# dangvansam/viet-asr

Hardware: AMD Instinct MI355X
Metric: real_time_factor (higher is better)
Workload: dtype f32 via 2xf16 split operands (22-bit significands, 3 f16 MFMA products per multiply, fp32 accumulate)

## Files before the change

viet-asr_amd/csrc/encoder_dw_mfma.hip:

```cpp
#include <cstdlib>

#include "vasr_internal.h"
#include "vasr_device.h"
#include <type_traits>

namespace vasr {

namespace {

using f32x4 = __attribute__((ext_vector_type(4))) float;
using v4f = __attribute__((ext_vector_type(4))) float;
using v2f = __attribute__((ext_vector_type(2))) float;
using f16x8 = __attribute__((ext_vector_type(8))) _Float16;
using f16x2 = __attribute__((ext_vector_type(2))) _Float16;
using u32x4 = __attribute__((vector_size(16))) unsigned int;

constexpr int kTile = 512;
constexpr int kGroup = 256;
constexpr int kUttPerWave = 8;
constexpr int kRowStages = 1;

template <int K, int DIL>
struct TzGeom {
  static constexpr int PAD = DIL > 1 ? (DIL * K) / 2 - 1 : K / 2;
  static constexpr int PADL = (PAD + 3) & ~3;
  static constexpr int OFF = PADL - PAD;
  static constexpr int SPAN = 15 + DIL * (K - 1) + OFF + 1;
  static constexpr int NS = (SPAN + 31) / 32;
  static constexpr int STAGES = kRowStages;
  static constexpr int TSZ = 32 * NS + 16;
  static constexpr int ROWS = kTile - 16 + 32 * NS;
  static constexpr int NLD = (ROWS / 4 + 63) / 64;
  static constexpr int PLANE = 2 * 256 * NLD;
  static constexpr int LDS_DATA = 2 * PLANE;
  static constexpr int LDS_TAB = 4 * TSZ;
  static constexpr int LDS_WAVE = LDS_DATA + LDS_TAB;
  static_assert(ROWS % 4 == 0 && LDS_WAVE % 16 == 0, "staging granularity");
};

__device__ __forceinline__ void wave_sync() {
  __builtin_amdgcn_fence(__ATOMIC_RELEASE, "wavefront");
  __builtin_amdgcn_wave_barrier();
  __builtin_amdgcn_fence(__ATOMIC_ACQUIRE, "wavefront");
}
__device__ __forceinline__ f32x4 mma(uint4 a, uint4 b, f32x4 c) {
  return __builtin_amdgcn_mfma_f32_16x16x32_f16(__builtin_bit_cast(f16x8, a), __builtin_bit_cast(f16x8, b), c, 0, 0, 0);
}
__device__ __forceinline__ float lane_pull(int src4, float v) {
  return __int_as_float(__builtin_amdgcn_ds_bpermute(src4, __float_as_int(v)));
}

template <int K, int DIL>
__global__ __launch_bounds__(256) void dw_toeplitz_kernel(const float* __restrict__ x, int64_t ldx,
                                                          const unsigned* __restrict__ taps,
                                                          const float* __restrict__ tap_inv,
                                                          const int32_t* __restrict__ lens_in,
                                                          const int32_t* __restrict__ lens_out,
                                                          const unsigned* __restrict__ amax_x, int amax_x_stride,
                                                          int amax_x_n, int channels, int batch,
                                                          float* __restrict__ y, int64_t ldy,
                                                          unsigned* __restrict__ amax_y, int amax_y_stride, int upw_nt,
                                                          int tiles, int n_rest) {
  using G = TzGeom<K, DIL>;
  const int bid = (int)blockIdx.x;
  const int rest = ((bid >> 3) / tiles) * 8 + (bid & 7);
  if (rest >= n_rest) return;
  const int ncg = channels >> 2;
  const int bx = rest % ncg, by = rest / ncg, bz = (bid >> 3) % tiles;
  const int upw = upw_nt;
  constexpr int NS = G::NS, NLD = G::NLD, kStages = G::STAGES;
  extern __shared__ __attribute__((aligned(16))) unsigned char lds_raw[];
  const int lane = threadIdx.x & 63;
  const int wave = __builtin_amdgcn_readfirstlane(threadIdx.x >> 6);
  unsigned char* base = lds_raw + wave * G::LDS_WAVE;
  unsigned char* dat = base;
  unsigned* tab = reinterpret_cast<unsigned*>(base + G::LDS_DATA);
  const int c = bx * 4 + wave;
  const int t_tile = bz * kTile;
  const int n16 = lane & 15, kg = lane >> 4;
  const int b_lo = by * upw;
  const int b_hi = min(b_lo + upw, batch);
  if (b_lo >= b_hi) return;
  const bool two = t_tile + kGroup < ldy;

  uint4 ah[NS], al[NS];
  const float w_inv = tap_inv[c];

  struct Stage { v4f r[NLD]; };
  const int n_ld = min(NLD, (min((int)ldy - t_tile, kTile) - 16 + 32 * NS + 255) / 256);
  int voff[NLD];
#pragma unroll
  for (int j = 0; j < NLD; ++j) {
    const int tau = 4 * (lane + 64 * j);
    voff[j] = tau < G::ROWS && j < n_ld ? 4 * (t_tile - G::PADL + tau) : (int)0x80000000u;
    if (j >= n_ld) {
      *reinterpret_cast<uint2*>(dat + 8 * lane + 512 * j) = make_uint2(0u, 0u);
      *reinterpret_cast<uint2*>(dat + G::PLANE + 8 * lane + 512 * j) = make_uint2(0u, 0u);
    }
  }
  const int n_utt = b_hi - b_lo;
  const int64_t row_stride = (int64_t)channels * ldx;
  const float* xrow0 = x + ((int64_t)b_lo * channels + c) * ldx;
  const int64_t yrow_stride = (int64_t)channels * ldy;
  float* yrow0 = y + ((int64_t)b_lo * channels + c) * ldy;
  int rng[kUttPerWave], lout[kUttPerWave];
#pragma unroll
  for (int u = 0; u < kUttPerWave; ++u) {
    const int b = min(b_lo + u, batch - 1);
    rng[u] = u < n_utt ? 4 * min(lens_in[b], (int)ldx) : 0;
    lout[u] = lens_out[b];
  }
  auto gload = [&](int u, Stage& sg) {
    const auto d = __builtin_amdgcn_make_buffer_rsrc(const_cast<float*>(xrow0 + u * row_stride), 0, rng[u], 0x00020000);
#pragma unroll
    for (int j = 0; j < NLD; ++j) {
      sg.r[j] = __builtin_bit_cast(v4f, __builtin_amdgcn_raw_buffer_load_b128(d, voff[j], 0, 0));
    }
  };
  auto sstore = [&](const Stage& sg, float sx) {
    unsigned char* ph = dat + 8 * lane;
#pragma unroll
    for (int j = 0; j < NLD; ++j) {
      if (j >= n_ld) continue;
      const v4f v = sg.r[j];
      const v2f a = {v.x * sx, v.y * sx}, b = {v.z * sx, v.w * sx};
      const f16x2 ha = __builtin_convertvector(a, f16x2), hb = __builtin_convertvector(b, f16x2);
      const f16x2 la = __builtin_convertvector(a - __builtin_convertvector(ha, v2f), f16x2);
      const f16x2 lb = __builtin_convertvector(b - __builtin_convertvector(hb, v2f), f16x2);
      *reinterpret_cast<uint2*>(ph + 512 * j) = make_uint2(__builtin_bit_cast(unsigned, ha), __builtin_bit_cast(unsigned, hb));
      *reinterpret_cast<uint2*>(ph + G::PLANE + 512 * j) = make_uint2(__builtin_bit_cast(unsigned, la), __builtin_bit_cast(unsigned, lb));
    }
  };

  const unsigned char* bb = dat + 32 * n16 + 16 * kg;
  const int pull = 4 * ((lane >> 2) + 16 * (lane & 3));
  const int slot = c * tiles + bz;

  float sxu[kUttPerWave], ixu[kUttPerWave];
  unsigned mxu[kUttPerWave];
#pragma unroll
  for (int u = 0; u < kUttPerWave; ++u) mxu[u] = 0u;
  auto publish = [&]() {
    if (!amax_y) return;
#define VASR_DPP(xx, ctrl) ((unsigned)__builtin_amdgcn_update_dpp(0, (int)(xx), (ctrl), 0xF, 0xF, false))
    const bool b0 = lane & 1, b1 = lane & 2, b2 = lane & 4;
    unsigned r[4], q[2];
#pragma unroll
    for (int k = 0; k < 4; ++k)
      r[k] = max(b0 ? mxu[2 * k + 1] : mxu[2 * k], VASR_DPP(b0 ? mxu[2 * k] : mxu[2 * k + 1], 0xB1));
#pragma unroll
    for (int k = 0; k < 2; ++k)
      q[k] = max(b1 ? r[2 * k + 1] : r[2 * k], VASR_DPP(b1 ? r[2 * k] : r[2 * k + 1], 0x4E));
    const unsigned send = b2 ? q[0] : q[1];
    unsigned m = max(b2 ? q[1] : q[0], max(VASR_DPP(send, 0x104), VASR_DPP(send, 0x114)));
    m = max(m, VASR_DPP(m, 0x128));
#undef VASR_DPP
    {
      const auto sw = __builtin_amdgcn_permlane16_swap(m, m, false, false);
      m = max((unsigned)sw[0], (unsigned)sw[1]);
    }
    {
      const auto sw = __builtin_amdgcn_permlane32_swap(m, m, false, false);
      m = max((unsigned)sw[0], (unsigned)sw[1]);
    }
    const auto da = __builtin_amdgcn_make_buffer_rsrc(amax_y + (int64_t)b_lo * amax_y_stride, 0, 4 * n_utt * amax_y_stride, 0x00020000);
    const int off = lane < kUttPerWave ? 4 * (lane * amax_y_stride + slot) : (int)0x80000000u;
    __builtin_amdgcn_raw_buffer_store_b32(m, da, off, 0, 0);
  };
  auto do_task = [&](auto u_tag, Stage& sg) {
    constexpr int u = decltype(u_tag)::value;
    sstore(sg, sxu[u]);
    if constexpr (u + kStages < kUttPerWave) gload(u + kStages, sg);
    wave_sync();

    f32x4 acc0 = {0.f, 0.f, 0.f, 0.f}, acc1 = {0.f, 0.f, 0.f, 0.f};
    constexpr bool kAllB = NS <= 3;
    auto load_b = [&](int q, uint4 (&bh)[NS], uint4 (&bl)[NS]) {
#pragma unroll
      for (int s = 0; s < NS; ++s) {
        bh[s] = *reinterpret_cast<const uint4*>(bb + 2 * kGroup * q + 64 * s);
        bl[s] = *reinterpret_cast<const uint4*>(bb + G::PLANE + 2 * kGroup * q + 64 * s);
      }
    };
    auto step = [&](f32x4 acc, int s, const uint4 (&bh)[NS], const uint4 (&bl)[NS]) {
      acc = mma(al[s], bh[s], acc);
      acc = mma(ah[s], bl[s], acc);
      acc = mma(ah[s], bh[s], acc);
      return acc;
    };
    {
      uint4 b0h[NS], b0l[NS], b1h[NS], b1l[NS];
      load_b(0, b0h, b0l);
      if (kAllB && two) {
        load_b(1, b1h, b1l);
#pragma unroll
        for (int s = 0; s < NS; ++s) {
          acc0 = step(acc0, s, b0h, b0l);
          acc1 = step(acc1, s, b1h, b1l);
        }
      } else {
#pragma unroll
        for (int s = 0; s < NS; ++s) acc0 = step(acc0, s, b0h, b0l);
        if (two) {
          load_b(1, b1h, b1l);
#pragma unroll
          for (int s = 0; s < NS; ++s) acc1 = step(acc1, s, b1h, b1l);
        }
      }
    }

    const float os = w_inv * ixu[u];
    const int lo = lout[u];
    float* yr = yrow0 + u * yrow_stride;
    const auto dy = __builtin_amdgcn_make_buffer_rsrc(yr, 0, 4 * (int)ldy, 0x00020000);
    v4f o0 = {acc0[0] * os, acc0[1] * os, acc0[2] * os, acc0[3] * os};
    v4f o1 = {acc1[0] * os, acc1[1] * os, acc1[2] * os, acc1[3] * os};
    o0.x = lane_pull(pull, o0.x); o0.y = lane_pull(pull, o0.y); o0.z = lane_pull(pull, o0.z); o0.w = lane_pull(pull, o0.w);
    o1.x = lane_pull(pull, o1.x); o1.y = lane_pull(pull, o1.y); o1.z = lane_pull(pull, o1.z); o1.w = lane_pull(pull, o1.w);
    float mx = 0.f;
    auto finish = [&](v4f o, int q) {
      const int tq = t_tile + kGroup * q;
      if (lo < tq + kGroup) {
        const int nv = lo - tq - 4 * lane;
        o.x = nv > 0 ? o.x : 0.f;
        o.y = nv > 1 ? o.y : 0.f;
        o.z = nv > 2 ? o.z : 0.f;
        o.w = nv > 3 ? o.w : 0.f;
      }
      mx = fmaxf(mx, fmaxf(fmaxf(fabsf(o.x), fabsf(o.y)), fmaxf(fabsf(o.z), fabsf(o.w))));
      __builtin_amdgcn_raw_buffer_store_b128(__builtin_bit_cast(u32x4, o), dy, 4 * (tq + 4 * lane), 0, 0);
    };
    finish(o0, 0);
    finish(o1, 1);
    mxu[u] = __float_as_uint(mx);
    wave_sync();
  };

  Stage stg[kStages];
#pragma unroll
  for (int i = 0; i < kStages; ++i) gload(i, stg[i]);

  constexpr int NTL = (G::TSZ + 63) / 64;
  unsigned tapv[NTL];
#pragma unroll
  for (int j = 0; j < NTL; ++j) tapv[j] = lane + 64 * j < G::TSZ ? taps[(int64_t)c * G::TSZ + lane + 64 * j] : 0u;

  {
    unsigned m[kUttPerWave];
    const unsigned* ap[kUttPerWave];
#pragma unroll
    for (int u = 0; u < kUttPerWave; ++u) {
      m[u] = 0u;
      ap[u] = amax_x + (int64_t)min(b_lo + u, b_hi - 1) * amax_x_stride;
    }
    for (int i0 = 0; i0 < amax_x_n; i0 += 64) {
      const int i = min(i0 + lane, amax_x_n - 1);
#pragma unroll
      for (int u = 0; u < kUttPerWave; ++u) m[u] = max(m[u], ap[u][i]);
    }
#pragma unroll
    for (int u = 0; u < kUttPerWave; ++u) f16_scale(wave_max_u32(m[u]), &sxu[u], &ixu[u]);
  }

#pragma unroll
  for (int j = 0; j < NTL; ++j)
    if (lane + 64 * j < G::TSZ) tab[lane + 64 * j] = tapv[j];
  wave_sync();
  {
    const unsigned* tp = tab + 15 - n16 + 8 * kg;
#pragma unroll
    for (int s = 0; s < NS; ++s) {
      unsigned v[8];
#pragma unroll
      for (int e = 0; e < 8; ++e) v[e] = tp[32 * s + e];
      ah[s] = make_uint4(__builtin_amdgcn_perm(v[1], v[0], 0x05040100u), __builtin_amdgcn_perm(v[3], v[2], 0x05040100u),
                         __builtin_amdgcn_perm(v[5], v[4], 0x05040100u), __builtin_amdgcn_perm(v[7], v[6], 0x05040100u));
      al[s] = make_uint4(__builtin_amdgcn_perm(v[1], v[0], 0x07060302u), __builtin_amdgcn_perm(v[3], v[2], 0x07060302u),
                         __builtin_amdgcn_perm(v[5], v[4], 0x07060302u), __builtin_amdgcn_perm(v[7], v[6], 0x07060302u));
    }
  }

  auto run = [&](auto u_tag, auto& self) -> void {
    constexpr int u = decltype(u_tag)::value;
    if constexpr (u < kUttPerWave) {
      if (u >= n_utt) return publish();
      do_task(u_tag, stg[u % kStages]);
      self(std::integral_constant<int, u + 1>{}, self);
    } else {
      publish();
    }
  };
  run(std::integral_constant<int, 0>{}, run);
}

template <int K, int DIL>
int launch_tz(const float* x, int64_t ldx, const unsigned* taps, const float* tap_inv, const int32_t* li, const int32_t* lo,
              AmaxTab amax_x, int batch, int channels, float* y, int64_t ldy, AmaxTab* amax_y, hipStream_t st) {
  using G = TzGeom<K, DIL>;
  auto kern = dw_toeplitz_kernel<K, DIL>;
  constexpr int lds = 4 * G::LDS_WAVE;
  const unsigned tiles = (unsigned)((ldy + kTile - 1) / kTile);
  const int upw_env = dev_switches().dw_upw;
  int upw = kUttPerWave;
  if (upw_env >= 1 && upw_env <= kUttPerWave) upw = upw_env;
  else
    while (upw > 2 && (int64_t)channels * ((batch + upw - 1) / upw) * tiles < 4096) upw /= 2;
  const int n_rest = (channels / 4) * ((batch + upw - 1) / upw);
  dim3 grid((unsigned)(((n_rest + 7) / 8) * 8) * tiles);
  if (amax_y) {
    amax_y->n = channels * (int)tiles;
    if (amax_y->n > amax_y->stride) return -1;
  }
  VASR_LAUNCH(kern, grid, dim3(256), lds, st, x, ldx, taps, tap_inv, li, lo, amax_x.p, amax_x.stride, amax_x.n, channels, batch,
              y, ldy, amax_y ? amax_y->p : nullptr, amax_y ? amax_y->stride : 0,
              upw, (int)tiles, n_rest);
  return 0;
}

template <int K, int DIL>
int table_size() { return TzGeom<K, DIL>::TSZ; }

}

int depthwise_mfma_table_size(int kernel, int dilation) {
  if (dilation == 2 && kernel == 87) return table_size<87, 2>();
  if (dilation != 1) return 0;
  switch (kernel) {
    case 33: return table_size<33, 1>();
    case 39: return table_size<39, 1>();
    case 51: return table_size<51, 1>();
    case 63: return table_size<63, 1>();
    case 75: return table_size<75, 1>();
    default: return 0;
  }
}

float pack_depthwise_taps_f16x2(const float* w, int kernel, int dilation, int tsz, unsigned* table) {
  const int pad = dilation > 1 ? (dilation * kernel) / 2 - 1 : kernel / 2;
  const int off = ((pad + 3) & ~3) - pad;
  float mx = 0.f;
  for (int k = 0; k < kernel; ++k) mx = fabsf(w[k]) > mx ? fabsf(w[k]) : mx;
  int e = (int)(__builtin_bit_cast(unsigned, mx) >> 23);
  e = e < 16 ? 16 : (e > 254 ? 254 : e);
  const float s = __builtin_bit_cast(float, (unsigned)(268 - e) << 23), inv = __builtin_bit_cast(float, (unsigned)(e - 14) << 23);
  for (int i = 0; i < tsz; ++i) {
    const int d = i - (15 + off);
    float v = 0.f;
    if (d >= 0 && d % dilation == 0 && d / dilation < kernel) v = w[d / dilation] * s;
    const _Float16 h = (_Float16)v;
    const _Float16 l = (_Float16)(v - (float)h);
    table[i] = (unsigned)__builtin_bit_cast(unsigned short, h) | ((unsigned)__builtin_bit_cast(unsigned short, l) << 16);
  }
  return inv;
}

int launch_depthwise_mfma(const float* x, int64_t ldx, const unsigned* taps, const float* tap_inv, const int32_t* lens_in,
                          const int32_t* lens_out, AmaxTab amax_x, int batch, int channels, int kernel, int dilation,
                          float* y, int64_t ldy, AmaxTab* amax_y, hipStream_t st) {
  const bool aligned = channels % 4 == 0 && ldx % 4 == 0 && ldy % 4 == 0 && ldx >= 4 &&
                       (reinterpret_cast<uintptr_t>(x) & 15) == 0 && (reinterpret_cast<uintptr_t>(y) & 15) == 0;
  if (!aligned || !taps || !amax_x.p || amax_x.n <= 0) return -1;
#define TZ(KK, DD) return launch_tz<KK, DD>(x, ldx, taps, tap_inv, lens_in, lens_out, amax_x, batch, channels, y, ldy, amax_y, st)
  if (dilation == 2 && kernel == 87) TZ(87, 2);
  if (dilation == 1) {
    switch (kernel) {
      case 33: TZ(33, 1);
      case 39: TZ(39, 1);
      case 51: TZ(51, 1);
      case 63: TZ(63, 1);
      case 75: TZ(75, 1);
      default: break;
    }
  }
#undef TZ
  return -1;
}

}
```

viet-asr_amd/csrc/vasr_api.cpp:

```cpp
#include <hip/hip_runtime.h>

#include <cmath>
#include <cstdarg>
#include <cstdio>
#include <cstdlib>
#include <cstring>
#include <map>
#include <string>
#include <algorithm>
#include <vector>

#include "vasr.h"
#include "vasr_devtools.h"
#include "vasr_internal.h"

using namespace vasr;

namespace vasr { thread_local LaunchProbe g_probe; }

namespace {

thread_local std::string g_err;

int fail(int code, const char* fmt, ...) {
  char buf[512];
  va_list ap;
  va_start(ap, fmt);
  vsnprintf(buf, sizeof buf, fmt, ap);
  va_end(ap);
  g_err = buf;
  return code;
}

#define HIP_TRY(expr)                                                                          \
  do {                                                                                         \
    hipError_t e_ = (expr);                                                                    \
    if (e_ != hipSuccess) return fail(VASR_ERR_HIP, "%s: %s", #expr, hipGetErrorString(e_)); \
  } while (0)

struct HostTensor {
  std::vector<float> data;
  std::vector<int64_t> shape;
};

struct ConvLayer {
  int cin = 0, cout = 0, kernel = 1, stride = 1, dilation = 1, pad = 0;
  int m_pad = 0;
  float* d_w = nullptr;
  unsigned short* d_w3 = nullptr;
  unsigned short* d_w16 = nullptr;
  float w16_inv = 1.f;
  unsigned int* d_taps = nullptr;
  float* d_tap_inv = nullptr;
  int tap_tsz = 0;
  float* d_ftaps = nullptr;
  float f_l1 = 0.f;
  float* d_scale = nullptr;
  float* d_shift = nullptr;
  int step = -1;
  int conv_cin = 0;
  int groups = 1;
};

struct SeLayer {
  float* d_w1 = nullptr;
  float* d_w2 = nullptr;
  int c = 0, hidden = 0;
};

struct NormLayer {
  float* d_gamma = nullptr;
  float* d_beta = nullptr;
  int32_t* d_group_of = nullptr;
  int32_t* d_members = nullptr;
  int c = 0, groups = 0;
};

struct SubBlock {
  bool separable = true;
  ConvLayer dw, pw;
  ConvLayer pw_bd;
  SeLayer se;
  NormLayer norm;
};

struct Block {
  vasr_block_desc d;
  std::vector<SubBlock> subs;
  bool has_res = false;
  ConvLayer res;
  bool fused_res = false;
  ConvLayer fused;
  int fused_k1 = 0;
  int first_step = 0;
  int pane = -1, pane_off = 0, pane_c = 0, dense_panes = 0;
  bool keep_input = false;
  bool res_pane0 = false;
  int se_r = 0;
  int groups = 1, heads = 0;
  int norm_g = 0;
  std::vector<NormLayer> res_norm;
  std::vector<SeLayer> res_se;
  std::vector<ConvLayer> res_panes;
  std::vector<int> res_pane_off;
};

size_t align_up(size_t v, size_t a) { return (v + a - 1) / a * a; }
constexpr int kDefaultGemmMode = 3;
int parse_gemm_mode(const char* s) {
  if (!s) return kDefaultGemmMode;
  if (!strcmp(s, "fp32")) return 0;
  if (!strcmp(s, "bf16x3")) return 1;
  if (!strcmp(s, "bf16x2")) return 2;
  if (!strcmp(s, "f16x2")) return 3;
  return kDefaultGemmMode;
}
constexpr int kMaxSlices = 4;
constexpr int kAmaxTabs = 4;

}

struct vasr_handle {
  bool has_frontend = false, has_encoder = false, has_decoder = false, finalized = false;
  vasr_frontend_desc fe{};
  std::vector<float> fe_window, fe_fb;
  int feat_in = 0, dec_feat_in = 0, num_classes = 0;
  std::vector<Block> blocks;
  int pane_c_max = 0;
  int se_c_max = 0;
  int norm_c_max = 0, norm_g_max = 0;
  std::vector<LenStep> steps;
  std::map<std::string, HostTensor> weights;
  std::vector<void*> dev_allocs;
  FrontendTables ft{};
  LenStep* d_steps = nullptr;
  ConvLayer dec;
  int c_mid_max = 0, c_last = 0;
  int slices = getenv("VASR_SLICES") ? atoi(getenv("VASR_SLICES")) : 1;
  bool slice_ready = false;
  bool row_independent = false;
  int busy_cus = 0;
  DevSwitches sw = dev_switches();
  int n_cu = 256;
  hipStream_t slice_stream[kMaxSlices] = {};
  hipEvent_t slice_done[kMaxSlices] = {}, slice_fork{};
  int gemm_mode = parse_gemm_mode(getenv("VASR_GEMM"));
  bool profiling = false;
  struct ProfRec { hipEvent_t a, b; int cls; double flops, bytes; };
  std::vector<ProfRec> prof;
  std::vector<hipEvent_t> ev_pool;
};

#ifdef VASR_DEVTOOLS
const vasr::DevSwitches& vasr::dev_switches() {
  static const DevSwitches sw = [] {
    DevSwitches s;
    auto num = [](const char* name, int dflt, std::initializer_list<int> allowed) {
      const char* e = getenv(name);
      if (!e) return dflt;
      const int v = atoi(e);
      for (int a : allowed) if (a == v) return v;
      fprintf(stderr, "vasr (devtools build): %s=%s is not a documented value -- refusing to guess\n", name, e);
      abort();
      return dflt;
    };
    s.pw3_tile = num("VASR_PW3_TILE", 0, {0, 1, 2, 3, 4, 5});
    s.pw_lat = num("VASR_PW_LAT", 1, {0, 1});
    s.dw_pair = num("VASR_DW_PAIR", 1, {0, 1}) != 0;
    s.dw_mfma = num("VASR_DW_MFMA", 1, {0, 1}) != 0;
    s.dw_upw = num("VASR_DW_UPW", 0, {0, 1, 2, 3, 4, 5, 6, 7, 8});
    s.fused = num("VASR_FUSED", 1, {0, 1}) != 0;
    s.fused_min_tiles = getenv("VASR_FUSED_MIN_TILES") ? atoi(getenv("VASR_FUSED_MIN_TILES")) : 0;
    s.fused_tile = num("VASR_FUSED_TILE", 0, {0, 64, 128});
    s.fused_residual = num("VASR_NO_FUSED_RESIDUAL", 0, {0, 1}) == 0;
    s.beam_group = num("VASR_BEAM_GROUP", -1, {-1, 0, 1, 4});
    s.no_grouped = num("VASR_NO_GROUPED", 0, {0, 1}) != 0;
    return s;
  }();
  return sw;
}
#endif

struct vasr_lm {
  BeamLm view{};
  std::vector<void*> allocs;
};

namespace {

template <class T>
int upload(vasr_handle* h, const std::vector<T>& v, T** out) {
  void* p = nullptr;
  HIP_TRY(hipMalloc(&p, std::max<size_t>(v.size() * sizeof(T), 16)));
  h->dev_allocs.push_back(p);
  HIP_TRY(hipMemcpy(p, v.data(), v.size() * sizeof(T), hipMemcpyHostToDevice));
  *out = static_cast<T*>(p);
  return 0;
}

int same_pad(int k, int stride, int dil, int* pad) {
  if (stride > 1 && dil > 1) return fail(VASR_ERR_INVALID, "Only stride OR dilation may be greater than 1");
  *pad = dil > 1 ? (dil * k) / 2 - 1 : k / 2;
  return 0;
}

int64_t conv_out_frames(int64_t t, const ConvLayer& c) {
  return (t + 2 * c.pad - (int64_t)c.dilation * (c.kernel - 1) - 1) / c.stride + 1;
}

const HostTensor* find(const vasr_handle* h, const std::string& key) {
  auto it = h->weights.find(key);
  return it == h->weights.end() ? nullptr : &it->second;
}

int need(const vasr_handle* h, const std::string& key, size_t numel, const HostTensor** out) {
  const HostTensor* t = find(h, key);
  if (!t) return fail(VASR_ERR_STATE, "missing weight '%s'", key.c_str());
  if (t->data.size() != numel)
    return fail(VASR_ERR_INVALID, "weight '%s' has %zu elements, expected %zu", key.c_str(), t->data.size(), numel);
  *out = t;
  return 0;
}

int fold_bn(vasr_handle* h, const std::string& prefix, int c, int c_pad, ConvLayer* L, const std::vector<int>* perm = nullptr) {
  const HostTensor *g, *b, *m, *v;
  int rc;
  if ((rc = need(h, prefix + ".weight", c, &g))) return rc;
  if ((rc = need(h, prefix + ".bias", c, &b))) return rc;
  if ((rc = need(h, prefix + ".running_mean", c, &m))) return rc;
  if ((rc = need(h, prefix + ".running_var", c, &v))) return rc;
  std::vector<float> sc(c_pad, 0.f), sh(c_pad, 0.f);
  for (int i = 0; i < c; ++i) {
    const float invstd = 1.0f / std::sqrt(v->data[i] + 1e-3f);
    const float alpha = g->data[i] * invstd;
    const int o = perm ? (*perm)[i] : i;
    sc[o] = alpha;
    sh[o] = b->data[i] - m->data[i] * alpha;
  }
  if ((rc = upload(h, sc, &L->d_scale))) return rc;
  return upload(h, sh, &L->d_shift);
}

int unit_affine(vasr_handle* h, int c, int c_pad, ConvLayer* L) {
  std::vector<float> sc(c_pad, 0.f), sh(c_pad, 0.f);
  std::fill_n(sc.begin(), c, 1.f);
  int rc;
  if ((rc = upload(h, sc, &L->d_scale))) return rc;
  return upload(h, sh, &L->d_shift);
}

int conv_affine(vasr_handle* h, int norm_g, const std::string& prefix, int c, int c_pad, ConvLayer* L,
                const std::vector<int>* perm = nullptr) {
  return norm_g ? unit_affine(h, c, c_pad, L) : fold_bn(h, prefix, c, c_pad, L, perm);
}

int load_norm(vasr_handle* h, const std::string& prefix, int c, int G, const std::vector<int>* perm, NormLayer* L) {
  const HostTensor *g, *b;
  int rc;
  if ((rc = need(h, prefix + ".weight", c, &g)) || (rc = need(h, prefix + ".bias", c, &b))) return rc;
  const int cpg = c / G;
  std::vector<float> gs(c), bs(c);
  std::vector<int32_t> group_of(c), members(c);
  for (int p = 0; p < c; ++p) {
    const int o = perm ? (*perm)[p] : p;
    gs[o] = g->data[p];
    bs[o] = b->data[p];
    group_of[o] = p / cpg;
    members[p] = o;
  }
  L->c = c;
  L->groups = G;
  h->norm_c_max = std::max(h->norm_c_max, c);
  h->norm_g_max = std::max(h->norm_g_max, G);
  if ((rc = upload(h, gs, &L->d_gamma)) || (rc = upload(h, bs, &L->d_beta)) || (rc = upload(h, group_of, &L->d_group_of)))
    return rc;
  return upload(h, members, &L->d_members);
}

std::vector<int> shuffle_perm(int c, int G) {
  std::vector<int> perm(c);
  const int mg = c / G;
  for (int p = 0; p < c; ++p) perm[p] = (p % mg) * G + p / mg;
  return perm;
}

int bn_affine(vasr_handle* h, const std::string& prefix, int c, std::vector<float>* alpha, std::vector<float>* beta) {
  const HostTensor *g, *b, *m, *v;
  int rc;
  if ((rc = need(h, prefix + ".weight", c, &g)) || (rc = need(h, prefix + ".bias", c, &b)) ||
      (rc = need(h, prefix + ".running_mean", c, &m)) || (rc = need(h, prefix + ".running_var", c, &v)))
    return rc;
  alpha->resize(c);
  beta->resize(c);
  for (int i = 0; i < c; ++i) {
    const float invstd = 1.0f / std::sqrt(v->data[i] + 1e-3f);
    (*alpha)[i] = g->data[i] * invstd;
    (*beta)[i] = b->data[i] - m->data[i] * (*alpha)[i];
  }
  return 0;
}

struct SumSrc { std::string w_key, bn; int k; };
int pack_sum_1x1(vasr_handle* h, const std::vector<SumSrc>& src, int cout, int k1_split, ConvLayer* L) {
  int K = 0, rc;
  for (const SumSrc& s : src) K += s.k;
  std::vector<float> w((size_t)cout * K), sh_sum(cout, 0.f);
  int off = 0;
  for (const SumSrc& s : src) {
    const HostTensor* ws;
    std::vector<float> a, b;
    if ((rc = need(h, s.w_key, (size_t)cout * s.k, &ws)) || (rc = bn_affine(h, s.bn, cout, &a, &b))) return rc;
    for (int m = 0; m < cout; ++m) {
      for (int k = 0; k < s.k; ++k) w[(size_t)m * K + off + k] = a[m] * ws->data[(size_t)m * s.k + k];
      sh_sum[m] += b[m];
    }
    off += s.k;
  }
  L->cin = K;
  L->cout = cout;
  L->m_pad = (int)align_up(cout, 128);
  std::vector<float> wt((size_t)K * L->m_pad, 0.f), sc(L->m_pad, 1.f), sh(L->m_pad, 0.f);
  pack_pointwise_weights(w.data(), cout, K, L->m_pad, wt.data());
  for (int m = 0; m < cout; ++m) sh[m] = sh_sum[m];
  if (pointwise_split_supported(L->m_pad, K, k1_split)) {
    std::vector<unsigned short> w3((size_t)K * L->m_pad * 3);
    pack_pointwise_weights_bf16x3(w.data(), cout, K, L->m_pad, w3.data());
    if ((rc = upload(h, w3, &L->d_w3))) return rc;
    std::vector<unsigned short> w16((size_t)K * L->m_pad * 2);
    L->w16_inv = pack_pointwise_weights_f16x2(w.data(), cout, K, L->m_pad, w16.data());
    if ((rc = upload(h, w16, &L->d_w16))) return rc;
  }
  if ((rc = upload(h, wt, &L->d_w)) || (rc = upload(h, sc, &L->d_scale))) return rc;
  return upload(h, sh, &L->d_shift);
}

int pack_conv_data(vasr_handle* h, const float* w, const std::string& key, int cout, int cin, int kernel, ConvLayer* L,
                   bool fp32 = true, bool split = true) {
  int rc;
  L->m_pad = (int)align_up(cout, 128);
  if (!conv_split_supported(L->m_pad, cin))
    return fail(VASR_ERR_UNSUPPORTED, "%s: in_channels %d of a %d-tap conv is not a multiple of 64", key.c_str(), cin, kernel);
  const int K = kernel * cin;
  L->cin = K;
  L->cout = cout;
  L->conv_cin = cin;
  std::vector<float> g((size_t)cout * K);
  pack_conv_gemm_weights(w, cout, cin, kernel, g.data());
  if (split) {
    std::vector<unsigned short> w3((size_t)K * L->m_pad * 3);
    pack_pointwise_weights_bf16x3(g.data(), cout, K, L->m_pad, w3.data());
    if ((rc = upload(h, w3, &L->d_w3))) return rc;
    std::vector<unsigned short> w16((size_t)K * L->m_pad * 2);
    L->w16_inv = pack_pointwise_weights_f16x2(g.data(), cout, K, L->m_pad, w16.data());
    if ((rc = upload(h, w16, &L->d_w16))) return rc;
  }
  if (!fp32) return 0;
  std::vector<float> wt((size_t)K * L->m_pad, 0.f);
  pack_pointwise_weights(g.data(), cout, K, L->m_pad, wt.data());
  return upload(h, wt, &L->d_w);
}

int pack_conv(vasr_handle* h, const std::string& key, int cout, int cin, int kernel, ConvLayer* L) {
  const HostTensor* w;
  int rc;
  if ((rc = need(h, key, (size_t)cout * cin * kernel, &w))) return rc;
  return pack_conv_data(h, w->data.data(), key, cout, cin, kernel, L);
}

int pack_pointwise_data(vasr_handle* h, const float* w, const std::string& key, int cout, int cin, ConvLayer* L,
                        bool fp32 = true, bool split = true) {
  int rc;
  if (cin % 64) return fail(VASR_ERR_UNSUPPORTED, "%s: in_channels %d is not a multiple of 64", key.c_str(), cin);
  L->cin = cin;
  L->cout = cout;
  L->m_pad = (int)align_up(cout, 128);
  if (split && pointwise_split_supported(L->m_pad, cin, 0)) {
    std::vector<unsigned short> w3((size_t)cin * L->m_pad * 3);
    pack_pointwise_weights_bf16x3(w, cout, cin, L->m_pad, w3.data());
    if ((rc = upload(h, w3, &L->d_w3))) return rc;
    std::vector<unsigned short> w16((size_t)cin * L->m_pad * 2);
    L->w16_inv = pack_pointwise_weights_f16x2(w, cout, cin, L->m_pad, w16.data());
    if ((rc = upload(h, w16, &L->d_w16))) return rc;
  }
  if (!fp32) return 0;
  std::vector<float> wt((size_t)cin * L->m_pad, 0.f);
  pack_pointwise_weights(w, cout, cin, L->m_pad, wt.data());
  return upload(h, wt, &L->d_w);
}

int pack_pointwise(vasr_handle* h, const std::string& key, int cout, int cin, ConvLayer* L) {
  const HostTensor* w;
  int rc;
  if ((rc = need(h, key, (size_t)cout * cin, &w))) return rc;
  return pack_pointwise_data(h, w->data.data(), key, cout, cin, L);
}

int pack_grouped(vasr_handle* h, const std::string& key, const std::string& bn, int cout, int cin, int kernel, int G, bool conv,
                 ConvLayer* L, ConvLayer* BD, int norm_g) {
  const HostTensor* w;
  int rc;
  const int cg = cin / G, mg = cout / G;
  if ((rc = need(h, key, (size_t)cout * cg * kernel, &w))) return rc;
  std::vector<float> dense((size_t)cout * cin * kernel, 0.f);
  const std::vector<int> perm = shuffle_perm(cout, G);
  for (int p = 0; p < cout; ++p) {
    const int g = p / mg, o = perm[p];
    for (int c = 0; c < cg; ++c)
      for (int t = 0; t < kernel; ++t)
        dense[((size_t)o * cin + g * cg + c) * kernel + t] = w->data[((size_t)p * cg + c) * kernel + t];
  }
  const bool grouped = !h->sw.no_grouped && grouped_split_supported(cout, cin, G);
  if ((rc = conv ? pack_conv_data(h, dense.data(), key, cout, cin, kernel, BD, true, !grouped)
                 : pack_pointwise_data(h, dense.data(), key, cout, cin, BD, true, !grouped)) ||
      (rc = conv_affine(h, norm_g, bn, cout, BD->m_pad, BD, &perm)))
    return rc;
  if (!grouped) {
    *L = *BD;
    *BD = ConvLayer{};
    return 0;
  }
  if ((rc = conv ? pack_conv_data(h, w->data.data(), key, cout, cg, kernel, L, false)
                 : pack_pointwise_data(h, w->data.data(), key, cout, cg, L, false)) ||
      (rc = conv_affine(h, norm_g, bn, cout, L->m_pad, L)))
    return rc;
  L->groups = G;
  return 0;
}

struct SubKeys { int conv, bn, se; };
std::vector<SubKeys> mconv_layout(const Block& B) {
  std::vector<SubKeys> out;
  int j = 0;
  for (int r = 0; r < B.d.repeat; ++r) {
    SubKeys k{j, j + (B.d.separable ? 2 : 1), -1};
    j = k.bn + 1 + (B.groups > 1 ? 1 : 0);
    if (r != B.d.repeat - 1) j += 2;
    if (B.se_r && !B.d.residual) k.se = j++;
    out.push_back(k);
  }
  return out;
}

std::vector<std::string> se_prefixes(const vasr_handle* h, size_t i) {
  const Block& B = h->blocks[i];
  std::vector<std::string> out;
  if (!B.se_r) return out;
  char key[160];
  if (B.d.residual) {
    const int panes = B.dense_panes >= 2 ? B.dense_panes : 1;
    for (int q = 0; q < panes; ++q) {
      snprintf(key, sizeof key, "encoder.%zu.res.%d.2", i, q);
      out.push_back(key);
    }
    return out;
  }
  for (const SubKeys& k : mconv_layout(B)) {
    snprintf(key, sizeof key, "encoder.%zu.mconv.%d", i, k.se);
    out.push_back(key);
  }
  return out;
}

int check_se(vasr_handle* h) {
  for (size_t i = 0; i < h->blocks.size(); ++i) {
    const Block& B = h->blocks[i];
    if (!B.se_r) continue;
    const int c = B.d.filters, hid = c / B.se_r;
    if (hid == 0)
      return fail(VASR_ERR_INVALID, "block %zu: se_reduction_ratio %d leaves no hidden unit of %d channels", i, B.se_r, c);
    if (!se_supported(c, hid))
      return fail(VASR_ERR_UNSUPPORTED, "block %zu: squeeze-and-excitation over %d channels (at most 1024)", i, c);
    const HostTensor* t;
    int rc;
// ... 1518 lines not shown
```

viet-asr_amd/csrc/vasr_internal.h:

```cpp
#pragma once
#include <hip/hip_runtime.h>
#include <atomic>
#include <hip/hip_ext.h>
#include <stdint.h>
#include <stdlib.h>

namespace vasr {

struct DevSwitches {
  int pw3_tile = 0;
  int pw_lat = 1;
  bool dw_pair = true;
  bool dw_mfma = true;
  int dw_upw = 0;
  bool fused = true;
  int fused_min_tiles = 0;
  int fused_tile = 0;
  bool fused_residual = true;
  int beam_group = -1;
  bool no_grouped = false;
};
#ifdef VASR_DEVTOOLS
const DevSwitches& dev_switches();
#else
inline const DevSwitches& dev_switches() { static constexpr DevSwitches k{}; return k; }
#endif

struct LaunchProbe { hipEvent_t start = nullptr, stop = nullptr; };
extern thread_local LaunchProbe g_probe;
#define VASR_LAUNCH(kern, grid, block, lds, st, ...)                                                       \
  do {                                                                                                     \
    if (::vasr::g_probe.start) {                                                                           \
      hipExtLaunchKernelGGL(kern, grid, block, lds, st, ::vasr::g_probe.start, ::vasr::g_probe.stop, 0,   \
                            __VA_ARGS__);                                                                  \
      ::vasr::g_probe.start = nullptr;                                                                     \
    } else {                                                                                               \
      hipLaunchKernelGGL(kern, grid, block, lds, st, __VA_ARGS__);                                         \
    }                                                                                                      \
  } while (0)

inline hipError_t dyn_lds_opt_in(const void* kernel, int bytes, std::atomic<uint64_t>& done) {
  int dev = 0;
  if (hipGetDevice(&dev) != hipSuccess) dev = 0;
  const uint64_t bit = 1ull << (dev & 63);
  if (done.load(std::memory_order_relaxed) & bit) return hipSuccess;
  const hipError_t e = hipFuncSetAttribute(kernel, hipFuncAttributeMaxDynamicSharedMemorySize, bytes);
  if (e == hipSuccess) done.fetch_or(bit, std::memory_order_relaxed);
  return e;
}

#define VASR_LAUNCH_PART(first, last, kern, grid, block, lds, st, ...)                                     \
  do {                                                                                                     \
    if (::vasr::g_probe.start) {                                                                           \
      hipExtLaunchKernelGGL(kern, grid, block, lds, st, (first) ? ::vasr::g_probe.start : nullptr,         \
                            (last) ? ::vasr::g_probe.stop : nullptr, 0, __VA_ARGS__);                      \
      if (last) ::vasr::g_probe.start = nullptr;                                                           \
    } else {                                                                                               \
      hipLaunchKernelGGL(kern, grid, block, lds, st, __VA_ARGS__);                                         \
    }                                                                                                      \
  } while (0)

constexpr int kTimeTile = 128;
static inline int64_t pad_frames(int64_t t) { return (t + kTimeTile - 1) / kTimeTile * kTimeTile; }


struct AmaxTab {
  unsigned int* p = nullptr;
  int stride = 0;
  int n = 0;
};

struct FrontendTables {
  const float* window;
  const float* tw256;
  const float* tw512;
  const float* mel_w;
  const int32_t* mel_lo;
  int32_t guard_clamp;
};
constexpr int kMelTaps = 32;

void launch_stft_logmel(const FrontendTables& tb, const void* wav, bool pcm16, int batch, int64_t samples,
                        const int64_t* row_len, int hop, float preemph, float log_guard, float* mel, int64_t mel_ld, int frames,
                        hipStream_t st);
void launch_seq_len(const int64_t* len, int batch, int hop, int64_t* seq, hipStream_t st);
void launch_normalize_all(float* mel, int64_t mel_ld, const int64_t* seq, int batch, int n_mels, int frames, hipStream_t st);
void launch_normalize(float* mel, int64_t mel_ld, const int64_t* seq, int batch, int n_mels, int frames,
                      int normalize, hipStream_t st);

struct LenStep { int32_t kernel, stride, dilation, pad; };
void launch_normalize_chain(float* mel, int64_t mel_ld, const int64_t* len, int hop, int batch, int n_mels, int frames,
                            int normalize, int64_t* seq, const LenStep* d_steps, int n_steps, int32_t* lens_tab,
                            float* enc_len, const int64_t* wav_len, int frames_cap, hipStream_t st);
void launch_len_chain(const int64_t* seq, int batch, const LenStep* d_steps, int n_steps, int32_t* lens_tab,
                      float* enc_len, hipStream_t st, const int64_t* wav_len = nullptr, int hop = 1, int frames_cap = 0);

void launch_repad(const float* src, int64_t src_ld, int rows, int frames, float* dst, int64_t dst_ld,
                  hipStream_t st);

int launch_depthwise(const float* x, int64_t ldx, int frames_in, const float* w, const int32_t* lens_in,
                     const int32_t* lens_out, int batch, int channels, int kernel, int stride, int dilation,
                     int pad, float* y, int64_t ldy, hipStream_t st, AmaxTab* amax_y = nullptr);
int depthwise_amax_slots(int channels, int64_t ldy);

int depthwise_mfma_table_size(int kernel, int dilation);
float pack_depthwise_taps_f16x2(const float* w, int kernel, int dilation, int tsz, unsigned int* table);
int launch_depthwise_mfma(const float* x, int64_t ldx, const unsigned int* taps, const float* tap_inv,
                          const int32_t* lens_in, const int32_t* lens_out, AmaxTab amax_x, int batch,
                          int channels, int kernel, int dilation, float* y, int64_t ldy, AmaxTab* amax_y,
                          hipStream_t st);

struct PwArgs {
  const float* wt;
  const float* x;
  const int32_t* lens;
  const float* x2;
  const int32_t* lens2;
  int32_t K1;
  int64_t ldx2;
  const float* scale;
  const float* shift;
  const float* res;
  float* y;
  int32_t M, K, batch;
  int64_t ldx, ldy, ldr;
  int32_t frames;
  int32_t store_cols;
  int32_t m_store;
  int32_t relu;
  const int32_t* zero_from;
  int32_t busy_cus;
  AmaxTab amax_x;
  AmaxTab amax_x2;
  float w_inv_scale;
  AmaxTab amax_y;
  const int32_t* lens_y;
  int32_t conv_cin, conv_stride, conv_dil, conv_pad;
  int64_t conv_cols;
  int64_t bsx;
  int32_t groups;
};
void launch_pointwise(const PwArgs& a, hipStream_t st);
void pack_pointwise_weights(const float* w, int cout, int cin, int m_pad, float* out);

bool pointwise_split_supported(int M, int K, int K1);
bool conv_split_supported(int M, int cin);
bool grouped_split_supported(int cout, int cin, int groups);
void pack_conv_gemm_weights(const float* w, int cout, int cin, int kernel, float* out);
double launch_mfma_sustained(int gemm_mode, int n_cu, int steps, float* sink, hipStream_t st);
int launch_pointwise_split(const PwArgs& a, int arith, hipStream_t st, int* amax_n = nullptr);
bool pointwise_latency_supported(int M, int K, int K1);
int launch_pointwise_latency(const PwArgs& a, hipStream_t st, int* amax_n);
int pointwise_amax_slots(int M, int64_t ld);
void pack_pointwise_weights_bf16x3(const float* w, int cout, int cin, int m_pad, unsigned short* out);
float pack_pointwise_weights_f16x2(const float* w, int cout, int cin, int m_pad, unsigned short* out);
void launch_amax(const float* x, int64_t ld, int rows, int frames, const int32_t* lens, int batch, AmaxTab* amax,
                 hipStream_t st, int64_t batch_stride = 0);

struct FusedLaunch {
  const float* x; int64_t ldx;
  const int32_t* lens_in; const int32_t* lens_out;
  const float* taps; float dw_l1;
  AmaxTab amax_x;
  const void* wt; float w_inv_scale;
  const float* scale; const float* shift;
  float* y; int64_t ldy; int32_t frames, relu;
  AmaxTab amax_y; const int32_t* lens_y;
  const float* x2; int64_t ldx2; const int32_t* lens2; AmaxTab amax_x2;
  int32_t batch, kernel;
  int32_t tile_cols;
};
bool fused_dwpw_supported(int channels, int cout, int kernel, int stride, int dilation);
static inline int fused_tile_choice(int64_t tiles128, int cus) {
  if (tiles128 <= 0 || cus <= 0) return 0;
  const int64_t rounds = (tiles128 + cus - 1) / cus;
  if (tiles128 >= 3 * (int64_t)cus / 4 && (double)tiles128 >= 0.8 * (double)(rounds * cus)) return 128;
  if (2 * tiles128 >= 3 * (int64_t)cus / 8 && 2 * tiles128 <= cus) return 64;
  return 0;
}
int fused_dwpw_taps_per_pair(int kernel);
float pack_fused_taps(const float* w, int channels, int kernel, float* out);
int launch_fused_dwpw(const FusedLaunch& f, hipStream_t st, int* amax_n);

struct SeLaunch {
  const float* x; float* y;
  int64_t ld, bs;
  int channels, hidden, batch, frames, store_cols;
  const int32_t* lens;
  const float* w1; const float* w2;
  float* sums; float* scale;
  const int32_t* zero_lens;
  int relu, accumulate;
  AmaxTab* amax_y; const int32_t* lens_y;
};
bool se_supported(int channels, int hidden);
int launch_se(const SeLaunch& a, hipStream_t st);

struct NormLaunch {
  const float* x; float* y; const float* add;
  int64_t ld, ld_add, bs;
  int channels, groups, batch, frames, store_cols;
  const int32_t* lens;
  const int32_t* group_of; const int32_t* members;
  const float* gamma; const float* beta;
  float* row_mean; float* row_m2;
  float* g_mean; float* g_rstd;
  const int32_t* zero_lens;
  int relu;
  AmaxTab* amax_y; const int32_t* lens_y;
};
bool norm_supported(int channels, int groups);
int launch_norm(const NormLaunch& a, hipStream_t st);

void launch_logsoftmax_argmax(const float* logits, int64_t row_ld, int64_t batch_stride, int batch, int frames,
                              int num_classes, float* logp, int64_t* pred, hipStream_t st);
void launch_argmax(const float* logp, int batch, int64_t frames, int num_classes, int64_t* pred, hipStream_t st);
void launch_ctc_collapse(const int64_t* pred, int batch, int64_t frames, int blank, int32_t* ids,
                         int32_t* id_len, hipStream_t st, const int64_t* wav_len = nullptr, int hop = 0,
                         const LenStep* steps = nullptr, int n_steps = 0);

void launch_pcm16_to_f32(const short* in, int64_t n, float* out, hipStream_t st);
void launch_resample(const float* x, int64_t ld_in, const int64_t* len_in, int batch, const float* table, int nwin,
                     int num_table, double ratio, float* y, int64_t ld_out, int64_t* len_out, hipStream_t st);

struct BeamLm {
  const void* vocab; int vcap;
  const void* ngram; int ncap;
  const void* trie; int tbuckets;
  int order, bos, eos, unk;
  float alpha, beta, unk_offset;
};
constexpr int kBeamMax = 128;
struct BeamNbest {
  int nbest;
  int32_t* count;
  double* logit;
  double* score;
};
int launch_beam_search_wave(const float* logp, int batch, int frames, int V1, int space_id, int beam_width,
                            float token_min_logp, float beam_prune_logp, const BeamLm* lm, unsigned int* bp,
                            int32_t* out_ids, int32_t* out_len, float* out_score, hipStream_t st,
                            const int32_t* row_frames = nullptr, const BeamNbest* nbest = nullptr);
int beam_wave_utts_per_workgroup(int batch);
int launch_beam_search_group(const float* logp, int batch, int frames, int V1, int space_id, int beam_width,
                             float token_min_logp, float beam_prune_logp, const BeamLm* lm, unsigned int* bp,
                             int32_t* out_ids, int32_t* out_len, float* out_score, hipStream_t st,
                             const int32_t* row_frames = nullptr, const BeamNbest* nbest = nullptr);
int beam_group_width(int batch);
size_t beam_wave_lds_bytes();
unsigned long long beam_hash_step(unsigned long long h, unsigned long long v);
unsigned long long beam_hash_init();

}
```

Baseline: 128,200.

## Double-buffer LDS staging in depthwise Toeplitz kernel to overlap store with MFMA

Adds a pipelined variant of the depthwise Toeplitz MFMA kernel that keeps two LDS staging buffers per wave. The next utterance's f16 split is stored while the current one's MFMA results are finished, removing one wave barrier per utterance and overlapping LDS writes, global loads and epilogue work. It also always runs both 256-column groups with unconditional masking, and sets a waves-per-EU hint. In exchange it doubles per-wave LDS data size, which can lower occupancy, and may do redundant MFMA work on tail tiles. The previous kernel stays available behind a devtools switch.

```diff
diff --git a/viet-asr_amd/csrc/encoder_dw_mfma.hip b/viet-asr_amd/csrc/encoder_dw_mfma.hip
--- a/viet-asr_amd/csrc/encoder_dw_mfma.hip
+++ b/viet-asr_amd/csrc/encoder_dw_mfma.hip
@@ -20,7 +20,7 @@
 constexpr int kUttPerWave = 8;
 constexpr int kRowStages = 1;
 
-template <int K, int DIL>
+template <int K, int DIL, int NBUF = 2>
 struct TzGeom {
   static constexpr int PAD = DIL > 1 ? (DIL * K) / 2 - 1 : K / 2;
   static constexpr int PADL = (PAD + 3) & ~3;
@@ -32,7 +32,7 @@
   static constexpr int ROWS = kTile - 16 + 32 * NS;
   static constexpr int NLD = (ROWS / 4 + 63) / 64;
   static constexpr int PLANE = 2 * 256 * NLD;
-  static constexpr int LDS_DATA = 2 * PLANE;
+  static constexpr int LDS_DATA = NBUF * 2 * PLANE;
   static constexpr int LDS_TAB = 4 * TSZ;
   static constexpr int LDS_WAVE = LDS_DATA + LDS_TAB;
   static_assert(ROWS % 4 == 0 && LDS_WAVE % 16 == 0, "staging granularity");
@@ -50,18 +50,18 @@
   return __int_as_float(__builtin_amdgcn_ds_bpermute(src4, __float_as_int(v)));
 }
 
-template <int K, int DIL>
-__global__ __launch_bounds__(256) void dw_toeplitz_kernel(const float* __restrict__ x, int64_t ldx,
-                                                          const unsigned* __restrict__ taps,
-                                                          const float* __restrict__ tap_inv,
-                                                          const int32_t* __restrict__ lens_in,
-                                                          const int32_t* __restrict__ lens_out,
-                                                          const unsigned* __restrict__ amax_x, int amax_x_stride,
-                                                          int amax_x_n, int channels, int batch,
-                                                          float* __restrict__ y, int64_t ldy,
-                                                          unsigned* __restrict__ amax_y, int amax_y_stride, int upw_nt,
-                                                          int tiles, int n_rest) {
-  using G = TzGeom<K, DIL>;
+#define VASR_TZ_PARAMS                                                                                                 \
+  const float *__restrict__ x, int64_t ldx, const unsigned *__restrict__ taps,            \
+      const float *__restrict__ tap_inv,  const int32_t *__restrict__ lens_in,                   \
+      const int32_t *__restrict__ lens_out, const unsigned *__restrict__ amax_x, int amax_x_stride, int amax_x_n,       \
+      int channels, int batch, float *__restrict__ y, int64_t ldy, unsigned *__restrict__ amax_y, int amax_y_stride,    \
+      int upw_nt, int tiles, int n_rest
+#define VASR_TZ_ARGS \
+  x, ldx, taps, tap_inv, lens_in, lens_out, amax_x, amax_x_stride, amax_x_n, channels, batch, y, ldy, amax_y, amax_y_stride, upw_nt, tiles, n_rest
+
+template <int K, int DIL, bool PIPE>
+__device__ __forceinline__ void dw_toeplitz_body(VASR_TZ_PARAMS) {
+  using G = TzGeom<K, DIL, PIPE ? 2 : 1>;
   const int bid = (int)blockIdx.x;
   const int rest = ((bid >> 3) / tiles) * 8 + (bid & 7);
   if (rest >= n_rest) return;
@@ -93,9 +93,10 @@
   for (int j = 0; j < NLD; ++j) {
     const int tau = 4 * (lane + 64 * j);
     voff[j] = tau < G::ROWS && j < n_ld ? 4 * (t_tile - G::PADL + tau) : (int)0x80000000u;
-    if (j >= n_ld) {
-      *reinterpret_cast<uint2*>(dat + 8 * lane + 512 * j) = make_uint2(0u, 0u);
-      *reinterpret_cast<uint2*>(dat + G::PLANE + 8 * lane + 512 * j) = make_uint2(0u, 0u);
+    if (!PIPE && j >= n_ld) {
+#pragma unroll
+      for (int p = 0; p < G::LDS_DATA / G::PLANE; ++p)
+        *reinterpret_cast<uint2*>(dat + p * G::PLANE + 8 * lane + 512 * j) = make_uint2(0u, 0u);
     }
   }
   const int n_utt = b_hi - b_lo;
@@ -117,11 +118,11 @@
       sg.r[j] = __builtin_bit_cast(v4f, __builtin_amdgcn_raw_buffer_load_b128(d, voff[j], 0, 0));
     }
   };
-  auto sstore = [&](const Stage& sg, float sx) {
-    unsigned char* ph = dat + 8 * lane;
+  auto sstore = [&](const Stage& sg, float sx, unsigned char* buf) {
+    unsigned char* ph = buf + 8 * lane;
 #pragma unroll
     for (int j = 0; j < NLD; ++j) {
-      if (j >= n_ld) continue;
+      if (!PIPE && j >= n_ld) continue;
       const v4f v = sg.r[j];
       const v2f a = {v.x * sx, v.y * sx}, b = {v.z * sx, v.w * sx};
       const f16x2 ha = __builtin_convertvector(a, f16x2), hb = __builtin_convertvector(b, f16x2);
@@ -167,19 +168,17 @@
     const int off = lane < kUttPerWave ? 4 * (lane * amax_y_stride + slot) : (int)0x80000000u;
     __builtin_amdgcn_raw_buffer_store_b32(m, da, off, 0, 0);
   };
-  auto do_task = [&](auto u_tag, Stage& sg) {
-    constexpr int u = decltype(u_tag)::value;
-    sstore(sg, sxu[u]);
-    if constexpr (u + kStages < kUttPerWave) gload(u + kStages, sg);
-    wave_sync();
-
-    f32x4 acc0 = {0.f, 0.f, 0.f, 0.f}, acc1 = {0.f, 0.f, 0.f, 0.f};
+  const bool mul_two = PIPE || two;
+  auto multiply = [&](const unsigned char* buf, f32x4& acc0, f32x4& acc1) {
+    acc0 = f32x4{0.f, 0.f, 0.f, 0.f};
+    acc1 = f32x4{0.f, 0.f, 0.f, 0.f};
     constexpr bool kAllB = NS <= 3;
+    const unsigned char* bq = buf + (bb - dat);
     auto load_b = [&](int q, uint4 (&bh)[NS], uint4 (&bl)[NS]) {
 #pragma unroll
       for (int s = 0; s < NS; ++s) {
-        bh[s] = *reinterpret_cast<const uint4*>(bb + 2 * kGroup * q + 64 * s);
-        bl[s] = *reinterpret_cast<const uint4*>(bb + G::PLANE + 2 * kGroup * q + 64 * s);
+        bh[s] = *reinterpret_cast<const uint4*>(bq + 2 * kGroup * q + 64 * s);
+        bl[s] = *reinterpret_cast<const uint4*>(bq + G::PLANE + 2 * kGroup * q + 64 * s);
       }
     };
     auto step = [&](f32x4 acc, int s, const uint4 (&bh)[NS], const uint4 (&bl)[NS]) {
@@ -188,27 +187,28 @@
       acc = mma(ah[s], bh[s], acc);
       return acc;
     };
-    {
-      uint4 b0h[NS], b0l[NS], b1h[NS], b1l[NS];
-      load_b(0, b0h, b0l);
-      if (kAllB && two) {
+    uint4 b0h[NS], b0l[NS], b1h[NS], b1l[NS];
+    load_b(0, b0h, b0l);
+    if (kAllB && mul_two) {
+      load_b(1, b1h, b1l);
+#pragma unroll
+      for (int s = 0; s < NS; ++s) {
+        acc0 = step(acc0, s, b0h, b0l);
+        acc1 = step(acc1, s, b1h, b1l);
+      }
+    } else {
+#pragma unroll
+      for (int s = 0; s < NS; ++s) acc0 = step(acc0, s, b0h, b0l);
+      if (mul_two) {
         load_b(1, b1h, b1l);
 #pragma unroll
-        for (int s = 0; s < NS; ++s) {
-          acc0 = step(acc0, s, b0h, b0l);
-          acc1 = step(acc1, s, b1h, b1l);
-        }
-      } else {
-#pragma unroll
-        for (int s = 0; s < NS; ++s) acc0 = step(acc0, s, b0h, b0l);
-        if (two) {
-          load_b(1, b1h, b1l);
-#pragma unroll
-          for (int s = 0; s < NS; ++s) acc1 = step(acc1, s, b1h, b1l);
-        }
-      }
-    }
-
+        for (int s = 0; s < NS; ++s) acc1 = step(acc1, s, b1h, b1l);
+      }
+    }
+  };
+
+  auto epilogue = [&](auto u_tag, f32x4 acc0, f32x4 acc1) {
+    constexpr int u = decltype(u_tag)::value;
     const float os = w_inv * ixu[u];
     const int lo = lout[u];
     float* yr = yrow0 + u * yrow_stride;
@@ -220,7 +220,13 @@
     float mx = 0.f;
     auto finish = [&](v4f o, int q) {
       const int tq = t_tile + kGroup * q;
-      if (lo < tq + kGroup) {
+      if constexpr (PIPE) {
+        const int nv = q == 1 && !two ? 0 : lo - tq - 4 * lane;
+        o.x = nv > 0 ? o.x : 0.f;
+        o.y = nv > 1 ? o.y : 0.f;
+        o.z = nv > 2 ? o.z : 0.f;
+        o.w = nv > 3 ? o.w : 0.f;
+      } else if (lo < tq + kGroup) {
         const int nv = lo - tq - 4 * lane;
         o.x = nv > 0 ? o.x : 0.f;
         o.y = nv > 1 ? o.y : 0.f;
@@ -233,6 +239,16 @@
     finish(o0, 0);
     finish(o1, 1);
     mxu[u] = __float_as_uint(mx);
+  };
+
+  auto do_task = [&](auto u_tag, Stage& sg) {
+    constexpr int u = decltype(u_tag)::value;
+    sstore(sg, sxu[u], dat);
+    if constexpr (u + kStages < kUttPerWave) gload(u + kStages, sg);
+    wave_sync();
+    f32x4 acc0, acc1;
+    multiply(dat, acc0, acc1);
+    epilogue(u_tag, acc0, acc1);
     wave_sync();
   };
 
@@ -280,25 +296,69 @@
     }
   }
 
-  auto run = [&](auto u_tag, auto& self) -> void {
-    constexpr int u = decltype(u_tag)::value;
-    if constexpr (u < kUttPerWave) {
-      if (u >= n_utt) return publish();
-      do_task(u_tag, stg[u % kStages]);
-      self(std::integral_constant<int, u + 1>{}, self);
-    } else {
-      publish();
-    }
-  };
-  run(std::integral_constant<int, 0>{}, run);
-}
+  if constexpr (!PIPE) {
+    auto run = [&](auto u_tag, auto& self) -> void {
+      constexpr int u = decltype(u_tag)::value;
+      if constexpr (u < kUttPerWave) {
+        if (u >= n_utt) return publish();
+        do_task(u_tag, stg[u % kStages]);
+        self(std::integral_constant<int, u + 1>{}, self);
+      } else {
+        publish();
+      }
+    };
+    run(std::integral_constant<int, 0>{}, run);
+  } else {
+    constexpr int kNoVmem = 0x1 | 0x2 | 0x4 | 0x8 | 0x80 | 0x100 | 0x200 | 0x400;
+    auto plane = [&](int u) { return dat + (u & 1) * 2 * G::PLANE; };
+    sstore(stg[0], sxu[0], plane(0));
+    gload(1, stg[0]);
+    wave_sync();
+    auto run = [&](auto u_tag, auto& self) -> void {
+      constexpr int u = decltype(u_tag)::value;
+      if constexpr (u < kUttPerWave) {
+        if (u >= n_utt) return publish();
+        f32x4 acc0, acc1;
+        multiply(plane(u), acc0, acc1);
+        if constexpr (u + 1 < kUttPerWave) {
+          sstore(stg[0], sxu[u + 1], plane(u + 1));
+          if constexpr (u + 2 < kUttPerWave) gload(u + 2, stg[0]);
+        }
+        __builtin_amdgcn_sched_barrier(kNoVmem);
+        epilogue(u_tag, acc0, acc1);
+        wave_sync();
+        self(std::integral_constant<int, u + 1>{}, self);
+      } else {
+        publish();
+      }
+    };
+    run(std::integral_constant<int, 0>{}, run);
+  }
+}
+
+template <int K, int DIL>
+__global__ __launch_bounds__(256) __attribute__((amdgpu_waves_per_eu(TzGeom<K, DIL>::NS <= 2 ? 6 : TzGeom<K, DIL>::NS <= 3 ? 5 : 4)))
+void dw_toeplitz_kernel(VASR_TZ_PARAMS) {
+  dw_toeplitz_body<K, DIL, true>(VASR_TZ_ARGS);
+}
+#ifdef VASR_DEVTOOLS
+template <int K, int DIL>
+__global__ __launch_bounds__(256) void dw_toeplitz_legacy_kernel(VASR_TZ_PARAMS) {
+  dw_toeplitz_body<K, DIL, false>(VASR_TZ_ARGS);
+}
+#endif
 
 template <int K, int DIL>
 int launch_tz(const float* x, int64_t ldx, const unsigned* taps, const float* tap_inv, const int32_t* li, const int32_t* lo,
               AmaxTab amax_x, int batch, int channels, float* y, int64_t ldy, AmaxTab* amax_y, hipStream_t st) {
-  using G = TzGeom<K, DIL>;
   auto kern = dw_toeplitz_kernel<K, DIL>;
-  constexpr int lds = 4 * G::LDS_WAVE;
+  int lds = 4 * TzGeom<K, DIL, 2>::LDS_WAVE;
+#ifdef VASR_DEVTOOLS
+  if (dev_switches().dw_tz_legacy) {
+    kern = dw_toeplitz_legacy_kernel<K, DIL>;
+    lds = 4 * TzGeom<K, DIL, 1>::LDS_WAVE;
+  }
+#endif
   const unsigned tiles = (unsigned)((ldy + kTile - 1) / kTile);
   const int upw_env = dev_switches().dw_upw;
   int upw = kUttPerWave;
diff --git a/viet-asr_amd/csrc/vasr_api.cpp b/viet-asr_amd/csrc/vasr_api.cpp
--- a/viet-asr_amd/csrc/vasr_api.cpp
+++ b/viet-asr_amd/csrc/vasr_api.cpp
@@ -169,6 +169,7 @@
     s.dw_pair = num("VASR_DW_PAIR", 1, {0, 1}) != 0;
     s.dw_mfma = num("VASR_DW_MFMA", 1, {0, 1}) != 0;
     s.dw_upw = num("VASR_DW_UPW", 0, {0, 1, 2, 3, 4, 5, 6, 7, 8});
+    s.dw_tz_legacy = num("VASR_DW_TZ_LEGACY", 0, {0, 1}) != 0;
     s.fused = num("VASR_FUSED", 1, {0, 1}) != 0;
     s.fused_min_tiles = getenv("VASR_FUSED_MIN_TILES") ? atoi(getenv("VASR_FUSED_MIN_TILES")) : 0;
     s.fused_tile = num("VASR_FUSED_TILE", 0, {0, 64, 128});
diff --git a/viet-asr_amd/csrc/vasr_internal.h b/viet-asr_amd/csrc/vasr_internal.h
--- a/viet-asr_amd/csrc/vasr_internal.h
+++ b/viet-asr_amd/csrc/vasr_internal.h
@@ -13,6 +13,7 @@
   bool dw_pair = true;
   bool dw_mfma = true;
   int dw_upw = 0;
+  bool dw_tz_legacy = false;
   bool fused = true;
   int fused_min_tiles = 0;
   int fused_tile = 0;
```

Result: no change. 128,600 (median of 6 runs) (+0.3%).
